# nghiahuynh-ai/Flamed-TTS

Hardware: AMD Instinct MI355X
Metric: latent frames/s (RTF at nsteps-denoiser=128) (higher is better)
Workload: dtype bf16; 1 GPU; BASELINE configs[1]: 1 utterance(s) x 400 frames (5.0 s audio) per GPU, nsteps-denoiser=128, bf16 (one persistent launch per solve); batch_per_gpu=1, frames=400, nfe=128, global_batch=1, parallelism=utterance-sharded x1 (no collectives)

## Files before the change

flamed-tts_amd/csrc/capi.cpp:

```cpp
#include <cstdarg>
#include <cstdio>
#include <cstring>
#include <mutex>

#include "common.hpp"
#include "flamed_hip.h"

namespace fl {
static thread_local char g_err[1024] = "";

void set_error(const char* fmt, ...) {
  va_list ap;
  va_start(ap, fmt);
  vsnprintf(g_err, sizeof(g_err), fmt, ap);
  va_end(ap);
}
const char* last_error() { return g_err; }

int device_of(const void* p, int* dev) {
  if (!p || !dev) return kBadArg;
  hipPointerAttribute_t a;
  if (hipPointerGetAttributes(&a, p) != hipSuccess) {
    (void)hipGetLastError();
    return kBadArg;
// ... 58 lines not shown
      {"dwgn_small", &Tune::dwgn_small, 0, 1, nullptr},
      {"fuse_euler", &Tune::fuse_euler, 0, 1, nullptr},
      {"pva_split", &Tune::pva_split, 0, 1, nullptr},
      {"persist", &Tune::persist, 0, 1, nullptr},
      {"split_batch", &Tune::split_batch, 1, 4, nullptr},
      {"split_graph", &Tune::split_graph, 0, 1, nullptr},
      {"split_prio", &Tune::split_prio, 0, 2, nullptr},
      {"prio_all", &Tune::prio_all, 0, 1, nullptr},
      {"split_min_rows", &Tune::split_min_rows, 1024, 1 << 30, nullptr},
      {"persist_opt", &Tune::persist_opt, 0, 1 << 20, nullptr},
      {"persist_seal_skip", &Tune::persist_seal_skip, -1, 1 << 20, nullptr},
      {"persist_inject", &Tune::persist_inject, -1, 1 << 20, nullptr},
      {"persist_multi", &Tune::persist_multi, 0, 1, nullptr},
      {"persist_pad", &Tune::persist_pad, 0, 1, nullptr},
      {"persist_pad_ntw", &Tune::persist_pad_ntw, 1, 8, nullptr},
      {"persist_multi_ntw", &Tune::persist_multi_ntw, 1, 8, nullptr},
      {"persist_ntw", &Tune::persist_ntw, 1, 8, nullptr},
      {"persist_capmode", &Tune::persist_capmode, 0, 1, nullptr},
      {"pva_persist", &Tune::pva_persist, 0, 1, nullptr},
      {"attn_mfma", &Tune::attn_mfma, 0, 1, nullptr},
      {"prior_split", &Tune::prior_split, 0, 1, nullptr},
      {"stop_after", &Tune::stop_after, -1, 1 << 20, nullptr},
      {"coop", &Tune::coop, 0, 1, nullptr},
      {"dwgn_var", &Tune::dwgn_var, 0, 2, nullptr},
      {"pva_stage", &Tune::pva_stage, 0, 3, nullptr},
      {"pva_inject", &Tune::pva_inject, -1, 1 << 20, nullptr},
  };
  for (const Knob& k : knobs) {
    if (std::strcmp(k.name, key) != 0) continue;
    int v = value;
// ... 30 lines not shown
```

flamed-tts_amd/csrc/common.hpp:

```cpp
#pragma once
#include <hip/hip_runtime.h>

#include <cstdint>
#include <cstdio>
#include <map>
#include <mutex>
#include <set>
#include <utility>
#include <vector>

namespace fl {

typedef __bf16 bf16;
typedef __bf16 bf16x8 __attribute__((ext_vector_type(8)));
typedef float f32x4 __attribute__((ext_vector_type(4)));
typedef unsigned int u32x4 __attribute__((ext_vector_type(4)));

void set_error(const char* fmt, ...);
const char* last_error();

enum Status : int {
  kOk = 0,
  kBadArg = 1001,
  kNoWorkspace = 1002,
// ... 126 lines not shown
  int x16 = 0;
  int g8p_rows = 12800;
  int dwgn = 1;
  int dwgn_small = 1;
  int fuse_euler = 1;
  int persist = 1;
  int split_batch = 2;
  int split_graph = 0;
  int prio_all = 0;
  int split_prio = 2;
  int split_min_rows = 6144;
  int persist_seal_skip = -1;
  int persist_inject = -1;
  int persist_pad = 1;
  int persist_pad_ntw = 4;
  int persist_multi = 1;
  int persist_ntw = 8;
  int persist_multi_ntw = 8;
  int persist_capmode = 0;
  int persist_opt = 885322;
  int pva_split = 0;
  int pva_persist = 1;
  int attn_mfma = 1;
  int prior_split = 1;
  int pva_stage = 1;
  int pva_inject = -1;
  int dwgn_var = 1;
  int coop = 1;
  int stop_after = -1;
};
// ... 165 lines not shown
```

flamed-tts_amd/csrc/denoiser.hip:

```cpp
#include <cstring>
#include "flamed_hip.h"
#include "flamed_diag.h"
#include "gemm.hpp"
#include "gemm_dma.hpp"
#include "gemm_8p.hpp"
#include "persist.hpp"

#include <mutex>
#include <string>
#include <vector>

namespace fl {

constexpr int kTinyRows = 320;

#ifdef FL_STAMPS
static unsigned long long* g_stamp_dev = nullptr;
static void stamp_select(int cls, hipStream_t st) {
  unsigned long long* p = (cls == tn().stamp_class) ? g_stamp_dev : nullptr;
  (void)hipMemcpyToSymbolAsync(HIP_SYMBOL(fl_stamp_buf), &p, sizeof(p), 0, hipMemcpyHostToDevice, st);
}
#else
static void stamp_select(int, hipStream_t) {}
#endif
// ... 1258 lines not shown
  if (idx >= R * dim) return;
  int r = idx / dim, j = idx - r * dim;
  int jj = j < half ? j : j - half;
  const float nl = -9.210340371976184f;
  float f = expf((nl * (float)jj) / (float)half);
  float a = t[r] * f;
  F[idx] = j < half ? cosf(a) : sinf(a);
}

__global__ void taps_t_kernel(const float* __restrict__ src, float* __restrict__ dst, int H, int KS) {
  const size_t i = (size_t)blockIdx.x * blockDim.x + threadIdx.x;
  if (i >= (size_t)H * KS) return;
  const int c = i / KS, j = i - (size_t)c * KS;
  dst[(size_t)j * H + c] = src[i];
}

__global__ void cast_kernel_bf16(const float* __restrict__ src, bf16* __restrict__ dst, size_t n) {
  size_t i = (size_t)blockIdx.x * blockDim.x + threadIdx.x;
  if (i < n) dst[i] = (bf16)src[i];
}
__global__ void copy_kernel_f32(const float* __restrict__ src, float* __restrict__ dst, size_t n) {
  size_t i = (size_t)blockIdx.x * blockDim.x + threadIdx.x;
  if (i < n) dst[i] = src[i];
}
template <typename DT>
__global__ void stack_taps_kernel(const float* __restrict__ src, DT* __restrict__ dst, int N, int Cin, int KT) {
  size_t i = (size_t)blockIdx.x * blockDim.x + threadIdx.x;
  size_t total = (size_t)N * Cin * KT;
  if (i >= total) return;
  int k = i % KT;
// ... 224 lines not shown
    return launch_gemm_cfg<32, 32, 3, DT>(al, W, ldw, ep, M, N, K, st);
  }
  if constexpr (std::is_same<DT, bf16>::value) {
    if (c == kCfgSmall && (tn().use_dma >= 2 || (tn().use_dma == 1 && AL::kSrcBytes == 2)))
      return launch_gemm_dma<32, 64>(al, W, ldw, ep, M, N, K, st);
  }
  return wide_a ? launch_gemm_auto<DT>(c, kWideA, al, W, ldw, ep, M, N, K, st) : launch_gemm_auto<DT>(c, al, W, ldw, ep, M, N, K, st);
}


struct DenBlockW {
  const void* w2; const void* w3; const void* m0; const void* m2;
  const unsigned char* q[4] = {nullptr, nullptr, nullptr, nullptr};
  const unsigned char* qs[4] = {nullptr, nullptr, nullptr, nullptr};
  const float *b2, *b3, *mb0, *mb2, *lnw, *lnb, *lnmw, *lnmb, *dww, *dwb, *gnw, *gnb;
};

struct Den {
  int C, H, NB, KS, S, dt;
  bool f8 = false;
  int MS;
  int MS0;
  int fold = 0;
  char* dev = nullptr;
  size_t dev_bytes = 0;
  float *t0w, *t0b, *t2w, *t2b, *cw, *cb, *adaw, *adab;
  void* win; const float* bin;
  std::vector<DenBlockW> blk;
  DenBlockW fin;
  void* wout; const float* bout;
// ... 278 lines not shown
  FL_ON_DEVICE(wdev);
  const int H = d->H, C = d->C, S = d->S, NB = d->NB, KS = d->KS;
  const size_t es = d->dt == FLAMED_BF16 ? 2 : 4;
  size_t off = 0;
  auto take = [&](size_t bytes) { size_t o = off; off = align256(off + bytes); return o; };
  size_t o_t0w = take(4ull * H * 256), o_t0b = take(4ull * H), o_t2w = take(4ull * H * H), o_t2b = take(4ull * H);
  size_t o_cw = take(4ull * H * S), o_cb = take(4ull * H);
  size_t o_adaw = take(4ull * d->MS0 * H), o_adab = take(4ull * d->MS0);
  size_t o_win = take(es * H * C);
  std::vector<size_t> o_blk(NB);
  for (int i = 0; i < NB; ++i) o_blk[i] = take(es * 4ull * H * H);
  size_t o_fin = take(es * 2ull * H * H);
  size_t o_out = take(es * (size_t)C * 3 * H);
  std::vector<size_t> o_dw(NB + 1);
  for (int i = 0; i <= NB; ++i) o_dw[i] = take(4ull * KS * H);
  const size_t n_vec = 1 + 11ull * NB + 5;
  const size_t o_vec = take(4ull * (n_vec * H + C));
  const size_t q_bytes = (size_t)H * H + mx_scale_bytes(H, H);
  const size_t o_q = d->f8 ? take(q_bytes * (4ull * NB + 2)) : 0;
  if (d->dev) { FL_HIP(hipFree(d->dev)); d->dev = nullptr; }
  FL_HIP(hipMalloc(&d->dev, off));
  d->dev_bytes = off;
  char* base = d->dev;
  auto cpy = [&](size_t o, const float* src, size_t n) -> int {
    hipLaunchKernelGGL(copy_kernel_f32, dim3((n + 255) / 256), dim3(256), 0, st, src, reinterpret_cast<float*>(base + o), n);
    FL_LAUNCH_CHECK();
    return kOk;
  };
  auto quant = [&](int slot, const float* src, const unsigned char** q, const unsigned char** qs) -> int {
    if (!d->f8) return kOk;
// ... 3 lines not shown
    FL_LAUNCH_CHECK();
    *q = p;
    *qs = p + (size_t)H * H;
    return kOk;
  };
  auto cast = [&](size_t o, const float* src, size_t n) -> int {
    if (d->dt == FLAMED_BF16) {
      hipLaunchKernelGGL(cast_kernel_bf16, dim3((n + 255) / 256), dim3(256), 0, st, src, reinterpret_cast<bf16*>(base + o), n);
      FL_LAUNCH_CHECK();
      return kOk;
    }
    return cpy(o, src, n);
  };
  int rc;
#define TRY(x) do { if ((rc = (x)) != kOk) return rc; } while (0)
  size_t vcur = o_vec;
  auto vec = [&](const float* src, size_t n, const float** dst) -> int {
    TRY(cpy(vcur, src, n));
    *dst = reinterpret_cast<const float*>(base + vcur);
    vcur += 4 * n;
    return kOk;
  };
  TRY(cpy(o_t0w, w[0], (size_t)H * 256)); TRY(cpy(o_t0b, w[1], H));
  TRY(cpy(o_t2w, w[2], (size_t)H * H)); TRY(cpy(o_t2b, w[3], H));
  TRY(cpy(o_cw, w[4], (size_t)H * S)); TRY(cpy(o_cb, w[5], H));
  TRY(cast(o_win, w[6], (size_t)H * C));
  d->t0w = (float*)(base + o_t0w); d->t0b = (float*)(base + o_t0b); d->t2w = (float*)(base + o_t2w); d->t2b = (float*)(base + o_t2b);
  d->cw = (float*)(base + o_cw); d->cb = (float*)(base + o_cb); d->adaw = (float*)(base + o_adaw); d->adab = (float*)(base + o_adab);
  d->win = base + o_win;
  TRY(vec(w[7], H, &d->bin));
// ... 2 lines not shown
    const float* const* bw = w + FLAMED_DEN_HEAD_W + FLAMED_DEN_BLOCK_W * i;
    TRY(cpy(o_adaw + 4ull * (size_t)i * 6 * H * H, bw[0], 6ull * H * H));
    TRY(cpy(o_adab + 4ull * (size_t)i * 6 * H, bw[1], 6ull * H));
    DenBlockW& B = d->blk[i];
    size_t ob = o_blk[i];
    TRY(cast(ob, bw[8], (size_t)H * H));
    TRY(cast(ob + es * H * H, bw[10], (size_t)H * H));
    TRY(cast(ob + 2 * es * H * H, bw[14], (size_t)H * H));
    TRY(cast(ob + 3 * es * H * H, bw[16], (size_t)H * H));
    B.w2 = base + ob; B.w3 = base + ob + es * H * H; B.m0 = base + ob + 2 * es * H * H; B.m2 = base + ob + 3 * es * H * H;
    TRY(quant(4 * i + 0, bw[8], &B.q[0], &B.qs[0])); TRY(quant(4 * i + 1, bw[10], &B.q[1], &B.qs[1]));
    TRY(quant(4 * i + 2, bw[14], &B.q[2], &B.qs[2])); TRY(quant(4 * i + 3, bw[16], &B.q[3], &B.qs[3]));
    hipLaunchKernelGGL(taps_t_kernel, dim3((H * KS + 255) / 256), dim3(256), 0, st, bw[4], reinterpret_cast<float*>(base + o_dw[i]), H, KS);
    FL_LAUNCH_CHECK();
    B.dww = reinterpret_cast<float*>(base + o_dw[i]);
    TRY(vec(bw[2], H, &B.lnw)); TRY(vec(bw[3], H, &B.lnb)); TRY(vec(bw[5], H, &B.dwb)); TRY(vec(bw[6], H, &B.gnw));
    TRY(vec(bw[7], H, &B.gnb)); TRY(vec(bw[9], H, &B.b2)); TRY(vec(bw[11], H, &B.b3)); TRY(vec(bw[12], H, &B.lnmw));
    TRY(vec(bw[13], H, &B.lnmb)); TRY(vec(bw[15], H, &B.mb0)); TRY(vec(bw[17], H, &B.mb2));
  }
  {
    const float* const* fw = w + FLAMED_DEN_HEAD_W + FLAMED_DEN_BLOCK_W * NB;
    TRY(cpy(o_adaw + 4ull * (size_t)NB * 6 * H * H, fw[0], 5ull * H * H));
    TRY(cpy(o_adab + 4ull * (size_t)NB * 6 * H, fw[1], 5ull * H));
    DenBlockW& F = d->fin;
    hipLaunchKernelGGL(taps_t_kernel, dim3((H * KS + 255) / 256), dim3(256), 0, st, fw[2], reinterpret_cast<float*>(base + o_dw[NB]), H, KS);
    FL_LAUNCH_CHECK();
    F.dww = reinterpret_cast<float*>(base + o_dw[NB]);
    TRY(vec(fw[3], H, &F.dwb)); TRY(vec(fw[4], H, &F.gnw)); TRY(vec(fw[5], H, &F.gnb));
    TRY(cast(o_fin, fw[6], (size_t)H * H)); TRY(vec(fw[7], H, &F.b2));
    TRY(cast(o_fin + es * H * H, fw[8], (size_t)H * H)); TRY(vec(fw[9], H, &F.b3));
    F.w2 = base + o_fin; F.w3 = base + o_fin + es * H * H;
    TRY(quant(4 * NB + 0, fw[6], &F.q[0], &F.qs[0])); TRY(quant(4 * NB + 1, fw[8], &F.q[1], &F.qs[1]));
    size_t n = (size_t)C * H * 3;
    if (d->dt == FLAMED_BF16)
      hipLaunchKernelGGL(stack_taps_kernel<bf16>, dim3((n + 255) / 256), dim3(256), 0, st, fw[10], reinterpret_cast<bf16*>(base + o_out), C, H, 3);
    else
      hipLaunchKernelGGL(stack_taps_kernel<float>, dim3((n + 255) / 256), dim3(256), 0, st, fw[10], reinterpret_cast<float*>(base + o_out), C, H, 3);
    FL_LAUNCH_CHECK();
    d->wout = base + o_out;
    TRY(vec(fw[11], C, &d->bout));
  }
#undef TRY
// ... 319 lines not shown
static size_t persist_layout(char* base, pk::Params* P) {
  size_t off = 0;
  auto take = [&](size_t bytes) { char* p = base ? base + off : nullptr; off = align256(off + bytes); return p; };
  const size_t T = pk::kMaxT, H = pk::kH, C = pk::kC;
  char* ctr = take(4 * (size_t)pk::kCtrInts);
  char* sticky = take(4 * (size_t)pk::kStickyInts);
  char* seal = take((size_t)pk::kWGs * 16);
  char* xp0 = take(T * pk::kSlots * 8);
  char* xp1 = take(T * pk::kSlots * 8);
  char* ximg = take(T * H * 4);
  char* a2 = take(T * H * 2);
  char* u = take(T * H * 2);
  char* xa = take(T * H * 2);
  char* xs = take(T * C * 2);
  char* gnp = take((size_t)pk::kGroups * H * 16);
  char* yb = take((size_t)pk::kWGs * 16 * 4);
  char* xbase = take(T * C * 4);
  if (P) {
    P->ctr = reinterpret_cast<int*>(ctr);
    P->sticky = reinterpret_cast<int*>(sticky);
    P->seal = reinterpret_cast<int*>(seal);
    P->xpart[0] = reinterpret_cast<float2*>(xp0);
    P->xpart[1] = reinterpret_cast<float2*>(xp1);
    P->ximg = reinterpret_cast<float*>(ximg);
    P->a2 = reinterpret_cast<bf16*>(a2);
    P->u = reinterpret_cast<bf16*>(u);
    P->xa = reinterpret_cast<bf16*>(xa);
    P->xs = reinterpret_cast<bf16*>(xs);
    P->gnp = reinterpret_cast<float4*>(gnp);
    P->yb = reinterpret_cast<float*>(yb);
    P->xbase = reinterpret_cast<float*>(xbase);
  }
  return off;
}

static int persist_alloc(Den* d, hipStream_t st) {
  if (d->pmem) return kOk;
  const size_t bytes = persist_layout(nullptr, nullptr);
  FL_HIP(hipMalloc(&d->pmem, bytes));
  FL_HIP(hipMemsetAsync(d->pmem, 0, bytes, st));
  FL_HIP(hipHostMalloc(reinterpret_cast<void**>(&d->pfail_host), 16, hipHostMallocDefault));
  *d->pfail_host = 0;
  FL_HIP(hipHostMalloc(reinterpret_cast<void**>(&d->perr_host), Den::kPRing * sizeof(int), hipHostMallocDefault));
  for (int i = 0; i < Den::kPRing; ++i) d->perr_host[i] = 0;
  d->pfails_seen = 0;
// ... 7 lines not shown

static void persist_poll_fails(Den* d) {
  if (!d->pfail_host) return;
  const int f = __atomic_load_n(d->pfail_host, __ATOMIC_RELAXED);
  if (f <= d->pfails_seen) return;
  d->pfails_seen = f;
  if (f >= Den::kPersistRetry && !d->pbroken) {
    d->pbroken = true;
    fprintf(stderr, "flamed: %d persistent solves failed (output NaN-poisoned); this handle uses the launch path from now on\n", f);
  } else {
    fprintf(stderr, "flamed: a persistent solve failed (%d of %d allowed); its output was NaN-poisoned\n", f, Den::kPersistRetry);
  }
}

static int persist_batch(int B) {
  if (B == 3) return 4;
  if (B >= 5 && B <= 7) return 8;
  return B;
}

static bool persist_eligible(Den* d, int B, int T) {
  const Tune& tu = tn();
  persist_poll_fails(d);
  if (!tu.persist || d->pbroken || d->dt != FLAMED_BF16 || d->f8 || !d->fold || !tu.lnfold) return false;
  if (d->H != pk::kH || d->C != pk::kC || d->NB > pk::kMaxNB || d->KS != pk::kTaps || T < 16) return false;
  const int B0 = B;
  if (B != 1 && tu.persist_multi && tu.persist_pad) B = persist_batch(B);
  if (B != 1 && (!tu.persist_multi || (B != 2 && B != 4 && B != 8))) return false;
  const int ntw = pk::persist_ntw(B, T, tu.persist_opt);
  if (B != B0 && 2 * B >= 3 * B0 && ntw > tu.persist_pad_ntw) return false;
  if (ntw > pk::kMaxNTW || ntw > tu.persist_ntw || ((tu.persist_opt & 1024) && ntw != 1)) return false;
  if (B > 1 && ntw > tu.persist_multi_ntw) return false;
  if (d->pdev_ok < 0) d->pdev_ok = pk::persist_device_ok(d->device) ? 1 : 0;
  return d->pdev_ok == 1;
}

struct Rk2 {
  double a;
  float dt, adt, c1, c2dt;
  Rk2(double a_, int nsteps) : a(a_) {
    const double h = 1.0 / (double)nsteps;
    dt = (float)h;
// ... 13 lines not shown
  const int Bp = tn().persist_pad ? persist_batch(B) : B;
  P.T = T; P.B = Bp; P.Bx = Bp != B ? B : 0; P.NB = d->NB; P.s0 = s0; P.s1 = s1;
  P.dt = (float)(1.0 / (double)nfe);
  if (rk) {
    P.rk2 = 1; P.dt = rk->dt; P.adt = rk->adt; P.c1 = rk->c1; P.c2dt = rk->c2dt;
  }
  P.mods = mods; P.MS = d->MS; P.MS0 = d->MS0;
  FL_REQUIRE(P.MS % 4 == 0 && P.MS0 % 4 == 0 && ((uintptr_t)mods & 15) == 0, "persistent solve: modulation rows not 16-B aligned");
  P.win = reinterpret_cast<const bf16*>(d->win); P.bin = d->bin;
  for (int i = 0; i <= d->NB; ++i) {
    const DenBlockW& b = i < d->NB ? d->blk[i] : d->fin;
    pk::BlockW& o = P.blk[i];
    o.w2 = reinterpret_cast<const bf16*>(b.w2); o.w3 = reinterpret_cast<const bf16*>(b.w3);
    o.m0 = i < d->NB ? reinterpret_cast<const bf16*>(b.m0) : nullptr;
    o.m2 = i < d->NB ? reinterpret_cast<const bf16*>(b.m2) : nullptr;
    o.b2 = b.b2; o.b3 = b.b3; o.dww = b.dww; o.dwb = b.dwb; o.gnw = b.gnw; o.gnb = b.gnb;
    if (i < d->NB) {
      o.mb0 = b.mb0; o.mb2 = b.mb2; o.lnw = b.lnw; o.lnb = b.lnb; o.lnmw = b.lnmw; o.lnmb = b.lnmb;
    }
  }
  P.wout = reinterpret_cast<const bf16*>(d->wout); P.bout = d->bout;
  P.xt = xt;
  P.tmo = 50000000;
  P.opt = tn().persist_opt;
  P.ntw = pk::persist_ntw(Bp, T, P.opt);
  P.inject_step = tn().persist_inject;
  P.seal_skip = tn().persist_seal_skip;
  hipEvent_t* ev = nullptr;
  const int slot = (int)(d->pring_n % Den::kPRing);
  if (!cap) {
// ... 531 lines not shown
```

flamed-tts_amd/csrc/persist.hip:

```cpp
#include <cstdio>
#include <cstdlib>

#include "flamed_hip.h"
#include "flamed_diag.h"
#include "persist.hpp"
#include "gemm_dma.hpp"

namespace fl {
namespace pk {

#ifdef FL_STAMPS
constexpr int kStampSlots = 160;
#define PST(step)                                                                                       \
  do {                                                                                                  \
    if ((step) == P.pst_step && P.pst && threadIdx.x == 0 && pst_k < kStampSlots)                       \
      P.pst[blockIdx.x * kStampSlots + pst_k] = __builtin_amdgcn_s_memrealtime();                      \
    ++pst_k;                                                                                            \
  } while (0)
#define PSTP(step) \
  (((step) == P.pst_step && P.pst && pst_k < kStampSlots) ? P.pst + blockIdx.x * kStampSlots + pst_k++ : (++pst_k, nullptr))
#define GND(k, v)                                                                                       \
  do {                                                                                                  \
    if (cur_step == P.gnd_step && P.gnd)                                                                \
      P.gnd[(((size_t)blk * kWGs + g * kSlots + s) * 32 + (tid & 31)) * 32 + (k)] = (v);                \
// ... 532 lines not shown

__device__ __forceinline__ void ld_cols(float (&v)[2][4], const float* p, int q) {
#pragma unroll
  for (int nt = 0; nt < 2; ++nt) {
    const float4 a = *reinterpret_cast<const float4*>(p + 16 * nt + 4 * q);
    v[nt][0] = a.x; v[nt][1] = a.y; v[nt][2] = a.z; v[nt][3] = a.w;
  }
}
__device__ __forceinline__ void fill_cols(float (&v)[2][4], float x) {
#pragma unroll
  for (int nt = 0; nt < 2; ++nt)
#pragma unroll
    for (int r = 0; r < 4; ++r) v[nt][r] = x;
}

__device__ __forceinline__ void row_stats(const float2* xpart, int T, int ra, int rb, int rbase, float* st) {
  const int n2 = 2 * (rb - ra);
  const __amdgpu_buffer_rsrc_t rs = rsrc(xpart, (unsigned)T * kSlots * 8);
  for (int idx = opq(threadIdx.x); idx < ((n2 + 63) & ~63); idx += kThreads) {
    const bool act = idx < n2;
    const int row = ra + (act ? idx >> 1 : 0), half = idx & 1;
    float mv[16], qv[16];
#pragma unroll
    for (int k = 0; k < 8; ++k) {
      const float4 v = as_f4(ld16(rs, (unsigned)((row * kSlots + half * 16 + 2 * k) * 8)));
      mv[2 * k] = v.x; qv[2 * k] = v.y; mv[2 * k + 1] = v.z; qv[2 * k + 1] = v.w;
    }
    float sm = 0.f;
#pragma unroll
    for (int k = 0; k < 16; ++k) sm += mv[k];
    sm = dpp_add<kDppXor1>(sm);
    const float mean = sm * (1.0f / kSlots);
    float m2 = 0.f;
#pragma unroll
    for (int k = 0; k < 16; ++k) {
      const float d = mv[k] - mean;
      m2 += qv[k] + (float)kCols * d * d;
    }
    m2 = dpp_add<kDppXor1>(m2);
    if (act && half == 0) {
      st[2 * (row - rbase)] = mean;
      st[2 * (row - rbase) + 1] = 1.0f / sqrtf(m2 * (1.0f / kH) + 1e-6f);
    }
  }
}

template <typename OT>
__device__ __forceinline__ void flush_tile(const char* stg, OT* dst, int ld, int r0, int ra, int rb, int col0, int T,
                                           bool local = false) {
  constexpr int CPR = kCols * (int)sizeof(OT) / 16;
  const __amdgpu_buffer_rsrc_t rs = rsrc(dst, (unsigned)T * ld * (unsigned)sizeof(OT));
  const int w16 = 16 * (threadIdx.x >> 6);
  for (int it = opq(threadIdx.x & 63); it < 16 * CPR; it += 64) {
    const int row = w16 + it / CPR, ch = it % CPR;
    if (row < ra || row >= rb) continue;
    const u32x4 v = *reinterpret_cast<const u32x4*>(stg + (row * kCols * sizeof(OT)) + ch * 16);
    const unsigned off = (unsigned)(((size_t)(r0 + row) * ld + col0) * sizeof(OT) + ch * 16);
    if (local) st16p(rs, off, v);
    else st16(rs, off, v);
// ... 35 lines not shown
__global__ __launch_bounds__(kThreads, 1) void den_persist_kernel(Params P) {
  extern __shared__ __attribute__((aligned(16))) char smem[];
  const int tid = threadIdx.x, lane = tid & 63;
  const int wave = __builtin_amdgcn_readfirstlane(tid >> 6);
  const int T = P.T;
  const int TT = P.B * P.T;
  const int H = kH;
  int g = blockIdx.x % kGroups, s = blockIdx.x / kGroups;
  if (P.opt & 8) {
    const int x = g, j = s;
    g = 4 * (x / 4) + (j % 4);
    s = 8 * (x % 4) + j / 4;
  }
  constexpr bool xloc = false;
  const bool frag = (P.opt & 64) != 0;
  const bool gran = (P.opt & 512) != 0;
  int r0, nr;
  group_rows(g, T, P.B, r0, nr, P.opt);
  const int gpu = kGroups / P.B, utt = g / gpu;
  const int ub = utt * T, ue = ub + T;
  const bool idle = P.Bx > 0 && utt >= P.Bx;
  const int MB = P.Bx > 0 ? P.Bx : P.B, mutt = idle ? P.Bx - 1 : utt;
  const int c = lane & 15, q = lane >> 4;
  const int col0 = kCols * s;
  char* stg = smem + L_HS;
  float* hs = reinterpret_cast<float*>(smem + L_HS);
  float* st = reinterpret_cast<float*>(smem + L_ST);
  float* red = reinterpret_cast<float*>(smem + L_RED);
  float4* gnv = reinterpret_cast<float4*>(smem + L_GNV);
  int* flag = reinterpret_cast<int*>(smem + L_FLAG);
// ... 150 lines not shown
    unsigned* const a1 = reinterpret_cast<unsigned*>(P.sticky + SY_ARRIVE1);
    unsigned* tk = reinterpret_cast<unsigned*>(smem + L_FLAG);
    if (tid == 0) tk[1] = __hip_atomic_fetch_add(a0, 1u, __ATOMIC_RELAXED, __HIP_MEMORY_SCOPE_AGENT);
    __syncthreads();
    const unsigned target = arrive_target(tk[1]);
    __syncthreads();
    const bool ok0 = arrive_wait(a0, target, tmo, flag);
    if (ok0) {
      if (tid < 4 && kCtrInts > 4 * (int)blockIdx.x + tid)
        __hip_atomic_store(P.ctr + 4 * blockIdx.x + tid, 0, __ATOMIC_RELAXED, __HIP_MEMORY_SCOPE_AGENT);
      if (tid < 4) __hip_atomic_store(P.seal + 4 * blockIdx.x + tid, 0, __ATOMIC_RELAXED, __HIP_MEMORY_SCOPE_AGENT);
      if (gran && tid < 32) {
        const __amdgpu_buffer_rsrc_t rq = rsrc(P.gnp, kGroups * kH * 16);
        st16(rq, (unsigned)((blockIdx.x * 32 + tid) * 16), u32x4{0u, 0u, 0u, 0u});
      }
      asm volatile("s_waitcnt vmcnt(0)" ::: "memory");
    }
    __syncthreads();
    if (tid == 0) __hip_atomic_fetch_add(a1, 1u, __ATOMIC_RELAXED, __HIP_MEMORY_SCOPE_AGENT);
    const bool ok1 = arrive_wait(a1, target, tmo, flag);
    if (!ok0 || !ok1) {
      if (tid == 0) {
        unsigned* pf = reinterpret_cast<unsigned*>(P.sticky + SY_PFAIL);
        if (__hip_atomic_exchange(pf, target, __ATOMIC_RELAXED, __HIP_MEMORY_SCOPE_AGENT) != target)
          __hip_atomic_fetch_add(fails, 1, __ATOMIC_RELAXED, __HIP_MEMORY_SCOPE_AGENT);
        __hip_atomic_store(errw, 5, __ATOMIC_RELAXED, __HIP_MEMORY_SCOPE_AGENT);
      }
      fail_exit();
      return;
    }
  }
  publish_xs();

  float X[NTW][2][4];

  for (int step = P.s0; step < P.s1; ++step) {
    const float* md = P.mods + (size_t)(step * MB + mutt) * P.MS;
    cur_step = step;
    if (step == P.inject_step) {
      if (tid == 0) raise_err(errw, fails, 3);
      fail_exit();
      return;
    }
#ifdef FL_STAMPS
    pst_k = 0;
#endif
    float binv[2][4];
// ... 26 lines not shown
      signal_dma<16>(mygrp);
    } else {
      signal(mygrp);
      next_w(P.blk[0].w2);
    }
    PST(step);
    ++L;

    for (int blk = 0; blk <= P.NB; ++blk) {
      const bool fin = blk == P.NB;
      const BlockW& bw = P.blk[blk];
      const float* mb = md + (size_t)blk * 6 * H;

      const int cc = tid & 31, rg = tid >> 5;
      float hsc[4], hsh[4], hlw[4], hlb[4], osc[2][4], osh[2][4], olw[2][4], olb[2][4];
#pragma unroll
      for (int e = 0; e < 4; ++e) {
        const int col = col0 + 4 * (tid & 7) + e;
        hsc[e] = mb[H + col];
        hsh[e] = mb[col];
        hlw[e] = fin ? 1.0f : bw.lnw[col];
        hlb[e] = fin ? 0.0f : bw.lnb[col];
      }
      ld_cols(osc, mb + H + col0, q);
      ld_cols(osh, mb + col0, q);
      if (fin) {
        fill_cols(olw, 1.0f);
        fill_cols(olb, 0.0f);
      } else {
        ld_cols(olw, bw.lnw + col0, q);
        ld_cols(olb, bw.lnb + col0, q);
      }
      float w[kTaps];
#pragma unroll
      for (int j = 0; j < kTaps; ++j) w[j] = bw.dww[(size_t)j * H + col0 + cc];
      const float dbias = bw.dwb[col0 + cc];
      float gwv = 0.f, gbv = 0.f;
      if (tid < kCols) {
        gwv = bw.gnw[col0 + tid];
        gbv = bw.gnb[col0 + tid];
      }
      PST(step);
      if (!wait_ge(errw, fails, tmo, grp, 16, kGroups, 32 * L, flag) || !seal_wait(0, kGroups)) { fail_exit(); return; }
      PST(step);
      float hva[4], hvb[4], ova[2][4], ovb[2][4];
#pragma unroll
      for (int e = 0; e < 4; ++e) {
        const float sc1 = 1.0f + hsc[e];
        hva[e] = fin ? sc1 : hlw[e] * sc1;
        hvb[e] = fin ? hsh[e] : hlb[e] * sc1 + hsh[e];
// ... 303 lines not shown
        signal(mygrp);
        if (fin) issue_out();
        else next_w(bw.m0);
      }
      PST(step);
      ++L;
      if (fin) break;

      const float* fo0 = md + P.MS0 + (size_t)blk * 2 * H;
      float fa0[2][4], fb0[2][4];
      ld_cols(fa0, fo0 + col0, q);
      ld_cols(fb0, fo0 + H + col0, q);
      PST(step);
      if (!wait_ge(errw, fails, tmo, mygrp, 0, 1, 32 * L, flag) || !seal_wait(g, 1)) { fail_exit(); return; }
      PST(step);
      row_stats(P.xpart[1], TT, r0, r0 + nr, r0 - kHalo, st);
      f32x4 accm_m0[NTW][2];
      if constexpr (KH) gemm_kh<kH>(P.xa, r0, nr, (smem + wb * kWPanel), accm_m0[0], wave, lane, PSTP(step), g, frag);
      else if constexpr (NTW == 1) gemm<kH>(P.xa, r0, nr, (smem + wb * kWPanel), accm_m0[0], wave, lane, PSTP(step), g, frag);
      else gemm_chunks<kH, NTW>(P.xa, r0, nr, (smem + wb * kWPanel), accm_m0, wave, lane, PSTP(step), g, frag, P.opt);
      PST(step);
#pragma unroll
      for (int ci = 0; ci < NTW; ++ci) {
        const int tl = wave + 4 * ci;
        const f32x4(&acc)[2] = accm_m0[ci];
        float v[2][4];
        const int p = 16 * tl + c + kHalo;
        const float mean = st[2 * p], rstd = st[2 * p + 1];
#pragma unroll
        for (int nt = 0; nt < 2; ++nt) {
#pragma unroll
          for (int i = 0; i < 4; ++i) v[nt][i] = silu(rstd * (acc[nt][i] - mean * fa0[nt][i]) + fb0[nt][i]);
        }
        if (16 * tl < nr) store_op_t(P.u, g, s, tl, v, r0, nr, col0, TT, lane, frag);
      }
      seal_put();
      if (dmafirst) {
        next_w(bw.m2);
        signal_dma<16>(mygrp);
      } else {
        signal(mygrp);
        next_w(bw.m2);
      }
// ... 40 lines not shown
    float fac[2][4], fbc[2][4];
    {
      const float* fo = md + P.MS0 + (size_t)P.NB * 2 * H;
#pragma unroll
      for (int nt = 0; nt < 2; ++nt) {
        const int n = 16 * nt + 4 * q, m = n < 24 ? n : n - 24;
        const int ns = (m >> 3) * kC + kCh * s + (m & 7);
        const float4 a = *reinterpret_cast<const float4*>(fo + ns), b = *reinterpret_cast<const float4*>(fo + 3 * kC + ns);
        fac[nt][0] = a.x; fac[nt][1] = a.y; fac[nt][2] = a.z; fac[nt][3] = a.w;
        fbc[nt][0] = b.x; fbc[nt][1] = b.y; fbc[nt][2] = b.z; fbc[nt][3] = b.w;
      }
    }
    PST(step);
    if (!wait_ge(errw, fails, tmo, mygrp, 0, 1, 32 * L, flag) || !seal_wait(g, 1)) { fail_exit(); return; }
    PST(step);
    row_stats(P.xpart[1], TT, r0, r0 + nr, r0 - kHalo, st);
    f32x4 acco[NTW][2];
    if constexpr (KH) gemm_kh<kH>(P.xa, r0, nr, (smem + wb * kWPanel), acco[0], wave, lane, PSTP(step), g, frag);
    else if constexpr (NTW == 1) gemm<kH>(P.xa, r0, nr, (smem + wb * kWPanel), acco[0], wave, lane, PSTP(step), g, frag);
    else gemm_chunks<kH, NTW>(P.xa, r0, nr, (smem + wb * kWPanel), acco, wave, lane, PSTP(step), g, frag, P.opt);
    PST(step);
    float* yl = reinterpret_cast<float*>(NTW == 1 ? stg : smem + wb * kWPanel);
    if (NTW > 1) __syncthreads();
#pragma unroll
    for (int ci = 0; ci < NTW; ++ci) {
      const int row = 16 * (wave + 4 * ci) + c, p = row + kHalo;
      if (NTW == 1 || row < nr) {
        const float mean = st[2 * p], rstd = st[2 * p + 1];
#pragma unroll
        for (int nt = 0; nt < 2; ++nt) {
          const int n0 = 16 * nt + 4 * q;
          if (n0 < 24) {
            float y[4];
#pragma unroll
            for (int i = 0; i < 4; ++i) y[i] = rstd * (acco[ci][nt][i] - mean * fac[nt][i]) + fbc[nt][i];
            *reinterpret_cast<float4*>(yl + row * 24 + n0) = make_float4(y[0], y[1], y[2], y[3]);
          }
        }
      }
    }
    __syncthreads();
    if (tid < 4 && nr > 0) {
      const __amdgpu_buffer_rsrc_t ry = rsrc(P.yb, kWGs * 16 * 4);
      const int half = tid >> 1, k = tid & 1;
      const float* src = half == 0 ? yl + (nr - 1) * 24 + 4 * k : yl + 16 + 4 * k;
      st16(ry, (unsigned)(((g + kGroups * s) * 16 + half * 8 + 4 * k) * 4), __builtin_bit_cast(u32x4, *reinterpret_cast<const float4*>(src)));
    }
    seal_put();
    if (dmafirst && step + 1 < P.s1) {
      next_win();
      signal_dma<4>(mygrp);
    } else {
      signal(mygrp);
      if (step + 1 < P.s1) next_win();
    }
    PST(step);
    ++L;

    PST(step);
    if (!wait_ge(errw, fails, tmo, grp, 16, kGroups, 32 * L, flag) || !seal_wait(0, kGroups)) { fail_exit(); return; }
    PST(step);
    int gp = 0, gn_ = 0;
    for (int k = 0; k < kGroups; ++k) {
      int a, b;
      group_rows(k, T, P.B, a, b, P.opt);
      if (b > 0 && a + b == r0) gp = k;
      if (b > 0 && a == r0 + nr) gn_ = k;
    }
#pragma unroll
    for (int ci = 0; ci < NTW; ++ci) {
      const int row = kChunk * ci + xr_row;
      if (row < nr) {
        const int t = r0 + row;
        const __amdgpu_buffer_rsrc_t ry = rsrc(P.yb, kWGs * 16 * 4);
        float vv[2];
#pragma unroll
        for (int e = 0; e < 2; ++e) {
          const int chl = 2 * (tid & 3) + e, ch = kCh * s + chl;
          float v = P.bout[ch] + yl[row * 24 + 8 + chl];
          if (t > ub) {
            const float y0 = row > 0 ? yl[(row - 1) * 24 + chl]
                                     : __builtin_bit_cast(float, __builtin_amdgcn_raw_buffer_load_b32(
                                           ry, (unsigned)(((gp + kGroups * s) * 16 + chl) * 4), 0, 16));
            v += y0;
          }
          if (t < ue - 1) {
            const float y2 = row < nr - 1 ? yl[(row + 1) * 24 + 16 + chl]
                                          : __builtin_bit_cast(float, __builtin_amdgcn_raw_buffer_load_b32(
                                                ry, (unsigned)(((gn_ + kGroups * s) * 16 + 8 + chl) * 4), 0, 16));
            v += y2;
          }
          vv[e] = v;
        }
        if constexpr (RK2) {
          float2* const stash = reinterpret_cast<float2*>(P.xbase + (size_t)t * kC + xch);
          if (!(step & 1)) {
            if constexpr (kStash) *stash = make_float2(xs0[ci], xs1[ci]);
            xs0[ci] = __fadd_rn(xs0[ci], __fmul_rn(P.adt, vv[0]));
            xs1[ci] = __fadd_rn(xs1[ci], __fmul_rn(P.adt, vv[1]));
          } else {
            float b0, b1;
            if constexpr (kStash) {
              const float2 b = *stash;
              b0 = b.x; b1 = b.y;
// ... 122 lines not shown
```

flamed-tts_amd/csrc/persist.hpp:

```cpp
#pragma once
#include "common.hpp"

namespace fl {
namespace pk {

constexpr int kGroups = 8, kSlots = 32, kWGs = kGroups * kSlots, kThreads = 256;
constexpr int kH = 1024, kC = 256, kCols = kH / kSlots, kCh = kC / kSlots;
constexpr int kChunk = 64, kMaxNTW = 8, kMaxRows = kChunk * kMaxNTW, kHalo = 15, kTaps = 31, kWin = kChunk + 2 * kHalo;
constexpr int kMaxNB = 8, kMaxT = kGroups * kMaxRows;
constexpr int kWPanel = kCols * kH * 2;
constexpr int kHsLd = kCols + 4;
constexpr int L_HS = 2 * kWPanel;
constexpr int L_ST = L_HS + kWin * kHsLd * 4;
constexpr int L_RED = L_ST + (kMaxRows + 2 * kHalo) * 8;
constexpr int L_GNV = L_RED + 8 * kCols * 4;
constexpr int L_FLAG = L_GNV + kCols * 16;
constexpr int kLds = (L_FLAG + 16 + 15) / 16 * 16;
static_assert(kLds <= 160 * 1024, "persistent solve LDS");
constexpr int CT_GRP = 0, CT_GN = 16 * kGroups, CT_ERR = CT_GN + 16 * kSlots, kCtrInts = CT_ERR + 16;
constexpr int SY_FAILS = 0, SY_ARRIVE0 = 32, SY_ARRIVE1 = 64, SY_PFAIL = 96, kStickyInts = 128;

__host__ __device__ inline unsigned arrive_target(unsigned ticket) {
  return ticket - ticket % (unsigned)kWGs + (unsigned)kWGs;
}
// ... 12 lines not shown
  const float* mods;
  int MS, MS0;
  const bf16* win;
  const float* bin;
  BlockW blk[kMaxNB + 1];
  const bf16* wout;
  const float* bout;
  float* xt;
  float2* xpart[2];
  float* ximg;
  bf16* a2;
  bf16* u;
  bf16* xa;
  bf16* xs;
  float4* gnp;
  float* yb;
  int* ctr;
  int* seal;
  int* sticky;
  int inject_step = -1;
  int seal_skip = -1;
  long long tmo;
  int ntw = 1;
  int opt = 0;
  unsigned long long* pst = nullptr;
  int pst_step = -1;
  float* gnd = nullptr;
  int gnd_step = -1;
  int rk2 = 0;
  float adt = 0.f, c1 = 0.f, c2dt = 0.f;
  float* xbase = nullptr;
};

bool persist_device_ok(int device);
inline int persist_ntw(int B, int T, int opt) {
  const int gpu = kGroups / B;
  int R = (T + gpu - 1) / gpu;
  if (opt & 2) R = ((T + 15) / 16 + gpu - 1) / gpu * 16;
  return (R + kChunk - 1) / kChunk;
}
int persist_launch(const Params& P, hipStream_t st, bool cooperative = true);

}
}
```

Measured before the change: 20400 latent frames/s.

## Replace group-wide barrier for output halo exchange with tagged per-neighbor atomics

The end-of-step output halo exchange no longer does a seal_put, a signal and a full wait across all groups. Each workgroup now publishes its boundary output rows as 64-bit tag+value atomics, and only the neighbor groups spin on those tags. The change also defers row-stat partial loads into registers for the NTW==1 path, so they overlap the GEMM instead of going through LDS. It adds a channel-major padded depthwise-tap copy for float4 loads, vectorises the modulation loads for NTW<=4, and adds an optional batch-padding knob. The spin-wait removes the global barrier but relies on tag ordering being correct, so a wrong tag could cause stale reads or hangs.

Result: faster. 21210 latent frames/s (median of 6 runs) (+4.0%).

```diff
diff --git a/flamed-tts_amd/csrc/capi.cpp b/flamed-tts_amd/csrc/capi.cpp
--- a/flamed-tts_amd/csrc/capi.cpp
+++ b/flamed-tts_amd/csrc/capi.cpp
@@ -96,6 +96,7 @@
       {"persist_multi", &Tune::persist_multi, 0, 1, nullptr},
       {"persist_pad", &Tune::persist_pad, 0, 1, nullptr},
       {"persist_pad_ntw", &Tune::persist_pad_ntw, 1, 8, nullptr},
+      {"persist_as", &Tune::persist_as, 0, 8, nullptr},
       {"persist_multi_ntw", &Tune::persist_multi_ntw, 1, 8, nullptr},
       {"persist_ntw", &Tune::persist_ntw, 1, 8, nullptr},
       {"persist_capmode", &Tune::persist_capmode, 0, 1, nullptr},
diff --git a/flamed-tts_amd/csrc/common.hpp b/flamed-tts_amd/csrc/common.hpp
--- a/flamed-tts_amd/csrc/common.hpp
+++ b/flamed-tts_amd/csrc/common.hpp
@@ -164,6 +164,7 @@
   int persist_inject = -1;
   int persist_pad = 1;
   int persist_pad_ntw = 4;
+  int persist_as = 0;
   int persist_multi = 1;
   int persist_ntw = 8;
   int persist_multi_ntw = 8;
diff --git a/flamed-tts_amd/csrc/denoiser.hip b/flamed-tts_amd/csrc/denoiser.hip
--- a/flamed-tts_amd/csrc/denoiser.hip
+++ b/flamed-tts_amd/csrc/denoiser.hip
@@ -1296,6 +1296,12 @@
   const int c = i / KS, j = i - (size_t)c * KS;
   dst[(size_t)j * H + c] = src[i];
 }
+__global__ void taps_cm_kernel(const float* __restrict__ src, float* __restrict__ dst, int H, int KS) {
+  const size_t i = (size_t)blockIdx.x * blockDim.x + threadIdx.x;
+  if (i >= (size_t)H * 32) return;
+  const int c = i / 32, j = i % 32;
+  dst[i] = j < KS ? src[(size_t)c * KS + j] : 0.f;
+}
 
 __global__ void cast_kernel_bf16(const float* __restrict__ src, bf16* __restrict__ dst, size_t n) {
   size_t i = (size_t)blockIdx.x * blockDim.x + threadIdx.x;
@@ -1550,6 +1556,7 @@
   const unsigned char* q[4] = {nullptr, nullptr, nullptr, nullptr};
   const unsigned char* qs[4] = {nullptr, nullptr, nullptr, nullptr};
   const float *b2, *b3, *mb0, *mb2, *lnw, *lnb, *lnmw, *lnmb, *dww, *dwb, *gnw, *gnb;
+  const float* dwc = nullptr;
 };
 
 struct Den {
@@ -1858,6 +1865,8 @@
   size_t o_out = take(es * (size_t)C * 3 * H);
   std::vector<size_t> o_dw(NB + 1);
   for (int i = 0; i <= NB; ++i) o_dw[i] = take(4ull * KS * H);
+  std::vector<size_t> o_dwc(NB + 1);
+  for (int i = 0; i <= NB; ++i) o_dwc[i] = take(4ull * 32 * H);
   const size_t n_vec = 1 + 11ull * NB + 5;
   const size_t o_vec = take(4ull * (n_vec * H + C));
   const size_t q_bytes = (size_t)H * H + mx_scale_bytes(H, H);
@@ -1891,6 +1900,14 @@
   };
   int rc;
 #define TRY(x) do { if ((rc = (x)) != kOk) return rc; } while (0)
+  auto taps_cm = [&](size_t o, const float* src, const float** dst) -> int {
+    *dst = nullptr;
+    if (KS > 32) return kOk;
+    hipLaunchKernelGGL(taps_cm_kernel, dim3((H * 32 + 255) / 256), dim3(256), 0, st, src, reinterpret_cast<float*>(base + o), H, KS);
+    FL_LAUNCH_CHECK();
+    *dst = reinterpret_cast<const float*>(base + o);
+    return kOk;
+  };
   size_t vcur = o_vec;
   auto vec = [&](const float* src, size_t n, const float** dst) -> int {
     TRY(cpy(vcur, src, n));
@@ -1923,6 +1940,7 @@
     hipLaunchKernelGGL(taps_t_kernel, dim3((H * KS + 255) / 256), dim3(256), 0, st, bw[4], reinterpret_cast<float*>(base + o_dw[i]), H, KS);
     FL_LAUNCH_CHECK();
     B.dww = reinterpret_cast<float*>(base + o_dw[i]);
+    TRY(taps_cm(o_dwc[i], bw[4], &B.dwc));
     TRY(vec(bw[2], H, &B.lnw)); TRY(vec(bw[3], H, &B.lnb)); TRY(vec(bw[5], H, &B.dwb)); TRY(vec(bw[6], H, &B.gnw));
     TRY(vec(bw[7], H, &B.gnb)); TRY(vec(bw[9], H, &B.b2)); TRY(vec(bw[11], H, &B.b3)); TRY(vec(bw[12], H, &B.lnmw));
     TRY(vec(bw[13], H, &B.lnmb)); TRY(vec(bw[15], H, &B.mb0)); TRY(vec(bw[17], H, &B.mb2));
@@ -1935,6 +1953,7 @@
     hipLaunchKernelGGL(taps_t_kernel, dim3((H * KS + 255) / 256), dim3(256), 0, st, fw[2], reinterpret_cast<float*>(base + o_dw[NB]), H, KS);
     FL_LAUNCH_CHECK();
     F.dww = reinterpret_cast<float*>(base + o_dw[NB]);
+    TRY(taps_cm(o_dwc[NB], fw[2], &F.dwc));
     TRY(vec(fw[3], H, &F.dwb)); TRY(vec(fw[4], H, &F.gnw)); TRY(vec(fw[5], H, &F.gnb));
     TRY(cast(o_fin, fw[6], (size_t)H * H)); TRY(vec(fw[7], H, &F.b2));
     TRY(cast(o_fin + es * H * H, fw[8], (size_t)H * H)); TRY(vec(fw[9], H, &F.b3));
@@ -2284,7 +2303,7 @@
   char* xa = take(T * H * 2);
   char* xs = take(T * C * 2);
   char* gnp = take((size_t)pk::kGroups * H * 16);
-  char* yb = take((size_t)pk::kWGs * 16 * 4);
+  char* yb = take((size_t)pk::kWGs * 2 * pk::kCh * 8);
   char* xbase = take(T * C * 4);
   if (P) {
     P->ctr = reinterpret_cast<int*>(ctr);
@@ -2298,7 +2317,7 @@
     P->xa = reinterpret_cast<bf16*>(xa);
     P->xs = reinterpret_cast<bf16*>(xs);
     P->gnp = reinterpret_cast<float4*>(gnp);
-    P->yb = reinterpret_cast<float*>(yb);
+    P->yb = reinterpret_cast<unsigned long long*>(yb);
     P->xbase = reinterpret_cast<float*>(xbase);
   }
   return off;
@@ -2336,6 +2355,8 @@
 }
 
 static int persist_batch(int B) {
+  const int as = tn().persist_as;
+  if ((as == 2 || as == 4 || as == 8) && B < as) return as;
   if (B == 3) return 4;
   if (B >= 5 && B <= 7) return 8;
   return B;
@@ -2347,7 +2368,7 @@
   if (!tu.persist || d->pbroken || d->dt != FLAMED_BF16 || d->f8 || !d->fold || !tu.lnfold) return false;
   if (d->H != pk::kH || d->C != pk::kC || d->NB > pk::kMaxNB || d->KS != pk::kTaps || T < 16) return false;
   const int B0 = B;
-  if (B != 1 && tu.persist_multi && tu.persist_pad) B = persist_batch(B);
+  if (tu.persist_multi && tu.persist_pad) B = persist_batch(B);
   if (B != 1 && (!tu.persist_multi || (B != 2 && B != 4 && B != 8))) return false;
   const int ntw = pk::persist_ntw(B, T, tu.persist_opt);
   if (B != B0 && 2 * B >= 3 * B0 && ntw > tu.persist_pad_ntw) return false;
@@ -2391,6 +2412,7 @@
     o.w2 = reinterpret_cast<const bf16*>(b.w2); o.w3 = reinterpret_cast<const bf16*>(b.w3);
     o.m0 = i < d->NB ? reinterpret_cast<const bf16*>(b.m0) : nullptr;
     o.m2 = i < d->NB ? reinterpret_cast<const bf16*>(b.m2) : nullptr;
+    P.dwc[i] = b.dwc;
     o.b2 = b.b2; o.b3 = b.b3; o.dww = b.dww; o.dwb = b.dwb; o.gnw = b.gnw; o.gnb = b.gnb;
     if (i < d->NB) {
       o.mb0 = b.mb0; o.mb2 = b.mb2; o.lnw = b.lnw; o.lnb = b.lnb; o.lnmw = b.lnmw; o.lnmb = b.lnmb;
diff --git a/flamed-tts_amd/csrc/persist.hip b/flamed-tts_amd/csrc/persist.hip
--- a/flamed-tts_amd/csrc/persist.hip
+++ b/flamed-tts_amd/csrc/persist.hip
@@ -570,35 +570,64 @@
     for (int r = 0; r < 4; ++r) v[nt][r] = x;
 }
 
+template <class PairAdd>
+__device__ __forceinline__ float2 combine_row_partials(const float (&mv)[16], const float (&qv)[16], PairAdd pair) {
+  float sm = 0.f;
+#pragma unroll
+  for (int k = 0; k < 16; ++k) sm += mv[k];
+  sm = pair(sm);
+  const float mean = sm * (1.0f / kSlots);
+  float m2 = 0.f;
+#pragma unroll
+  for (int k = 0; k < 16; ++k) {
+    const float d = mv[k] - mean;
+    m2 += qv[k] + (float)kCols * d * d;
+  }
+  m2 = pair(m2);
+  return make_float2(mean, 1.0f / sqrtf(m2 * (1.0f / kH) + 1e-6f));
+}
+__device__ __forceinline__ void unpack_row_partials(const u32x4 (&v)[8], float (&mv)[16], float (&qv)[16]) {
+#pragma unroll
+  for (int k = 0; k < 8; ++k) {
+    const float4 f = as_f4(v[k]);
+    mv[2 * k] = f.x; qv[2 * k] = f.y; mv[2 * k + 1] = f.z; qv[2 * k + 1] = f.w;
+  }
+}
+
 __device__ __forceinline__ void row_stats(const float2* xpart, int T, int ra, int rb, int rbase, float* st) {
   const int n2 = 2 * (rb - ra);
   const __amdgpu_buffer_rsrc_t rs = rsrc(xpart, (unsigned)T * kSlots * 8);
   for (int idx = opq(threadIdx.x); idx < ((n2 + 63) & ~63); idx += kThreads) {
     const bool act = idx < n2;
     const int row = ra + (act ? idx >> 1 : 0), half = idx & 1;
+    u32x4 v[8];
+#pragma unroll
+    for (int k = 0; k < 8; ++k) v[k] = ld16(rs, (unsigned)((row * kSlots + half * 16 + 2 * k) * 8));
     float mv[16], qv[16];
-#pragma unroll
-    for (int k = 0; k < 8; ++k) {
-      const float4 v = as_f4(ld16(rs, (unsigned)((row * kSlots + half * 16 + 2 * k) * 8)));
-      mv[2 * k] = v.x; qv[2 * k] = v.y; mv[2 * k + 1] = v.z; qv[2 * k + 1] = v.w;
-    }
-    float sm = 0.f;
-#pragma unroll
-    for (int k = 0; k < 16; ++k) sm += mv[k];
-    sm = dpp_add<kDppXor1>(sm);
-    const float mean = sm * (1.0f / kSlots);
-    float m2 = 0.f;
-#pragma unroll
-    for (int k = 0; k < 16; ++k) {
-      const float d = mv[k] - mean;
-      m2 += qv[k] + (float)kCols * d * d;
-    }
-    m2 = dpp_add<kDppXor1>(m2);
+    unpack_row_partials(v, mv, qv);
+    const float2 ms = combine_row_partials(mv, qv, [](float x) { return dpp_add<kDppXor1>(x); });
     if (act && half == 0) {
-      st[2 * (row - rbase)] = mean;
-      st[2 * (row - rbase) + 1] = 1.0f / sqrtf(m2 * (1.0f / kH) + 1e-6f);
-    }
-  }
+      st[2 * (row - rbase)] = ms.x;
+      st[2 * (row - rbase) + 1] = ms.y;
+    }
+  }
+}
+
+__device__ __forceinline__ void load_row_partials(u32x4 (&v)[8], const float2* xpart, int T, int r0, int nr, int tile,
+                                                  int lane_in) {
+  const int lane = opq(lane_in);
+  const int c = lane & 15, q = lane >> 4, row = 16 * tile + c;
+  const __amdgpu_buffer_rsrc_t rs = rsrc(xpart, (unsigned)T * kSlots * 8);
+  const unsigned base = q < 2 && row < nr ? (unsigned)(((r0 + row) * kSlots + q * 16) * 8) : 0x7ff00000u;
+#pragma unroll
+  for (int k = 0; k < 8; ++k) v[k] = ld16(rs, base + 16 * k);
+}
+__device__ __forceinline__ float2 finish_row_partials(const u32x4 (&v)[8], int lane_in) {
+  float mv[16], qv[16];
+  unpack_row_partials(v, mv, qv);
+  const float2 ms = combine_row_partials(mv, qv, [](float x) { return x + __shfl_xor(x, 16); });
+  const int c = lane_in & 15;
+  return make_float2(__shfl(ms.x, c), __shfl(ms.y, c));
 }
 
 template <typename OT>
@@ -664,6 +693,7 @@
   }
   constexpr bool xloc = false;
   const bool frag = (P.opt & 64) != 0;
+  constexpr bool kDefer = NTW == 1 && !KH;
   const bool gran = (P.opt & 512) != 0;
   int r0, nr;
   group_rows(g, T, P.B, r0, nr, P.opt);
@@ -844,6 +874,10 @@
         const __amdgpu_buffer_rsrc_t rq = rsrc(P.gnp, kGroups * kH * 16);
         st16(rq, (unsigned)((blockIdx.x * 32 + tid) * 16), u32x4{0u, 0u, 0u, 0u});
       }
+      if (tid < 8) {
+        const __amdgpu_buffer_rsrc_t ry = rsrc(P.yb, kWGs * 2 * kCh * 8);
+        st16(ry, (unsigned)((blockIdx.x * 8 + tid) * 16), u32x4{0u, 0u, 0u, 0u});
+      }
       asm volatile("s_waitcnt vmcnt(0)" ::: "memory");
     }
     __syncthreads();
@@ -861,6 +895,16 @@
     }
   }
   publish_xs();
+
+  unsigned long long* const ybq = P.yb;
+  int gp = 0, gn_ = 0;
+  for (int k = 0; k < kGroups; ++k) {
+    int a, b;
+    group_rows(k, T, P.B, a, b, P.opt);
+    if (b > 0 && a + b == r0) gp = k;
+    if (b > 0 && a == r0 + nr) gn_ = k;
+  }
+  const bool ynb_p = !idle && nr > 0 && r0 > ub, ynb_n = !idle && nr > 0 && r0 + nr < ue;
 
   float X[NTW][2][4];
 
@@ -917,13 +961,28 @@
 
       const int cc = tid & 31, rg = tid >> 5;
       float hsc[4], hsh[4], hlw[4], hlb[4], osc[2][4], osh[2][4], olw[2][4], olb[2][4];
-#pragma unroll
-      for (int e = 0; e < 4; ++e) {
-        const int col = col0 + 4 * (tid & 7) + e;
-        hsc[e] = mb[H + col];
-        hsh[e] = mb[col];
-        hlw[e] = fin ? 1.0f : bw.lnw[col];
-        hlb[e] = fin ? 0.0f : bw.lnb[col];
+      constexpr bool kWide = NTW <= 4;
+      if constexpr (!kWide) {
+#pragma unroll
+        for (int e = 0; e < 4; ++e) {
+          const int col = col0 + 4 * (tid & 7) + e;
+          hsc[e] = mb[H + col];
+          hsh[e] = mb[col];
+          hlw[e] = fin ? 1.0f : bw.lnw[col];
+          hlb[e] = fin ? 0.0f : bw.lnb[col];
+        }
+      } else {
+        const int col = col0 + 4 * (tid & 7);
+        const float4 a = *reinterpret_cast<const float4*>(mb + H + col), b = *reinterpret_cast<const float4*>(mb + col);
+        hsc[0] = a.x; hsc[1] = a.y; hsc[2] = a.z; hsc[3] = a.w;
+        hsh[0] = b.x; hsh[1] = b.y; hsh[2] = b.z; hsh[3] = b.w;
+        float4 lw = make_float4(1.0f, 1.0f, 1.0f, 1.0f), lb = make_float4(0.0f, 0.0f, 0.0f, 0.0f);
+        if (!fin) {
+          lw = *reinterpret_cast<const float4*>(bw.lnw + col);
+          lb = *reinterpret_cast<const float4*>(bw.lnb + col);
+        }
+        hlw[0] = lw.x; hlw[1] = lw.y; hlw[2] = lw.z; hlw[3] = lw.w;
+        hlb[0] = lb.x; hlb[1] = lb.y; hlb[2] = lb.z; hlb[3] = lb.w;
       }
       ld_cols(osc, mb + H + col0, q);
       ld_cols(osh, mb + col0, q);
@@ -935,8 +994,18 @@
         ld_cols(olb, bw.lnb + col0, q);
       }
       float w[kTaps];
-#pragma unroll
-      for (int j = 0; j < kTaps; ++j) w[j] = bw.dww[(size_t)j * H + col0 + cc];
+      if constexpr (kWide) {
+        const float4* wp = reinterpret_cast<const float4*>(P.dwc[blk] + (size_t)(col0 + cc) * 32);
+#pragma unroll
+        for (int j = 0; j < 8; ++j) {
+          const float4 t = wp[j];
+          w[4 * j] = t.x; w[4 * j + 1] = t.y; w[4 * j + 2] = t.z;
+          if (4 * j + 3 < kTaps) w[4 * j + 3] = t.w;
+        }
+      } else {
+#pragma unroll
+        for (int j = 0; j < kTaps; ++j) w[j] = bw.dww[(size_t)j * H + col0 + cc];
+      }
       const float dbias = bw.dwb[col0 + cc];
       float gwv = 0.f, gbv = 0.f;
       if (tid < kCols) {
@@ -1270,7 +1339,9 @@
       PST(step);
       if (!wait_ge(errw, fails, tmo, mygrp, 0, 1, 32 * L, flag) || !seal_wait(g, 1)) { fail_exit(); return; }
       PST(step);
-      row_stats(P.xpart[1], TT, r0, r0 + nr, r0 - kHalo, st);
+      [[maybe_unused]] u32x4 rp_m0[8];
+      if constexpr (kDefer) load_row_partials(rp_m0, P.xpart[1], TT, r0, nr, wave, lane);
+      else row_stats(P.xpart[1], TT, r0, r0 + nr, r0 - kHalo, st);
       f32x4 accm_m0[NTW][2];
       if constexpr (KH) gemm_kh<kH>(P.xa, r0, nr, (smem + wb * kWPanel), accm_m0[0], wave, lane, PSTP(step), g, frag);
       else if constexpr (NTW == 1) gemm<kH>(P.xa, r0, nr, (smem + wb * kWPanel), accm_m0[0], wave, lane, PSTP(step), g, frag);
@@ -1281,8 +1352,16 @@
         const int tl = wave + 4 * ci;
         const f32x4(&acc)[2] = accm_m0[ci];
         float v[2][4];
-        const int p = 16 * tl + c + kHalo;
-        const float mean = st[2 * p], rstd = st[2 * p + 1];
+        float mean, rstd;
+        if constexpr (kDefer) {
+          const float2 ms = finish_row_partials(rp_m0, lane);
+          mean = ms.x;
+          rstd = ms.y;
+        } else {
+          const int p = 16 * tl + c + kHalo;
+          mean = st[2 * p];
+          rstd = st[2 * p + 1];
+        }
 #pragma unroll
         for (int nt = 0; nt < 2; ++nt) {
 #pragma unroll
@@ -1353,7 +1432,9 @@
     PST(step);
     if (!wait_ge(errw, fails, tmo, mygrp, 0, 1, 32 * L, flag) || !seal_wait(g, 1)) { fail_exit(); return; }
     PST(step);
-    row_stats(P.xpart[1], TT, r0, r0 + nr, r0 - kHalo, st);
+    [[maybe_unused]] u32x4 rp_out[8];
+    if constexpr (kDefer) load_row_partials(rp_out, P.xpart[1], TT, r0, nr, wave, lane);
+    else row_stats(P.xpart[1], TT, r0, r0 + nr, r0 - kHalo, st);
     f32x4 acco[NTW][2];
     if constexpr (KH) gemm_kh<kH>(P.xa, r0, nr, (smem + wb * kWPanel), acco[0], wave, lane, PSTP(step), g, frag);
     else if constexpr (NTW == 1) gemm<kH>(P.xa, r0, nr, (smem + wb * kWPanel), acco[0], wave, lane, PSTP(step), g, frag);
@@ -1365,7 +1446,15 @@
     for (int ci = 0; ci < NTW; ++ci) {
       const int row = 16 * (wave + 4 * ci) + c, p = row + kHalo;
       if (NTW == 1 || row < nr) {
-        const float mean = st[2 * p], rstd = st[2 * p + 1];
+        float mean, rstd;
+        if constexpr (kDefer) {
+          const float2 ms = finish_row_partials(rp_out, lane);
+          mean = ms.x;
+          rstd = ms.y;
+        } else {
+          mean = st[2 * p];
+          rstd = st[2 * p + 1];
+        }
 #pragma unroll
         for (int nt = 0; nt < 2; ++nt) {
           const int n0 = 16 * nt + 4 * q;
@@ -1379,54 +1468,64 @@
       }
     }
     __syncthreads();
-    if (tid < 4 && nr > 0) {
-      const __amdgpu_buffer_rsrc_t ry = rsrc(P.yb, kWGs * 16 * 4);
-      const int half = tid >> 1, k = tid & 1;
-      const float* src = half == 0 ? yl + (nr - 1) * 24 + 4 * k : yl + 16 + 4 * k;
-      st16(ry, (unsigned)(((g + kGroups * s) * 16 + half * 8 + 4 * k) * 4), __builtin_bit_cast(u32x4, *reinterpret_cast<const float4*>(src)));
-    }
-    seal_put();
-    if (dmafirst && step + 1 < P.s1) {
-      next_win();
-      signal_dma<4>(mygrp);
-    } else {
-      signal(mygrp);
-      if (step + 1 < P.s1) next_win();
-    }
+    const unsigned ytag = (unsigned)(step - P.s0 + 1);
+    if (tid < 2 * kCh && nr > 0 && !idle) {
+      const float y = tid < kCh ? yl[(nr - 1) * 24 + tid] : yl[16 + tid - kCh];
+      __hip_atomic_store(ybq + (size_t)(g + kGroups * s) * (2 * kCh) + tid, ((unsigned long long)ytag << 32) | __float_as_uint(y),
+                         __ATOMIC_RELAXED, __HIP_MEMORY_SCOPE_AGENT);
+    }
+    if (step + 1 < P.s1) next_win();
     PST(step);
-    ++L;
 
     PST(step);
-    if (!wait_ge(errw, fails, tmo, grp, 16, kGroups, 32 * L, flag) || !seal_wait(0, kGroups)) { fail_exit(); return; }
+    if (ynb_p || ynb_n) {
+      if (tid < 64) {
+        const bool need = tid < kCh ? ynb_p : tid < 2 * kCh && ynb_n;
+        const unsigned long long* yq = ybq + (size_t)((tid < kCh ? gp : gn_) + kGroups * s) * (2 * kCh) + (tid & (2 * kCh - 1));
+        float y = 0.f;
+        bool ok = true;
+        const unsigned long long t0 = __builtin_amdgcn_s_memrealtime();
+        for (unsigned it = 0;; ++it) {
+          bool mine = true;
+          if (need) {
+            const unsigned long long a = __hip_atomic_load(yq, __ATOMIC_RELAXED, __HIP_MEMORY_SCOPE_AGENT);
+            mine = (unsigned)(a >> 32) == ytag;
+            y = __uint_as_float((unsigned)a);
+          }
+          if (__all(mine)) break;
+          if ((it & 31) == 31) {
+            if (__hip_atomic_load(errw, __ATOMIC_RELAXED, __HIP_MEMORY_SCOPE_AGENT) != 0) { ok = false; break; }
+            if ((long long)(__builtin_amdgcn_s_memrealtime() - t0) > tmo) {
+              if (tid == 0) raise_err(errw, fails, 1);
+              ok = false;
+              break;
+            }
+          }
+          __builtin_amdgcn_s_sleep(1);
+        }
+        if (tid == 0) *flag = ok ? 1 : 0;
+        if (tid < 2 * kCh) red[tid] = y;
+      }
+      __syncthreads();
+      if (*flag == 0) { fail_exit(); return; }
+    }
     PST(step);
-    int gp = 0, gn_ = 0;
-    for (int k = 0; k < kGroups; ++k) {
-      int a, b;
-      group_rows(k, T, P.B, a, b, P.opt);
-      if (b > 0 && a + b == r0) gp = k;
-      if (b > 0 && a == r0 + nr) gn_ = k;
-    }
 #pragma unroll
     for (int ci = 0; ci < NTW; ++ci) {
       const int row = kChunk * ci + xr_row;
       if (row < nr) {
         const int t = r0 + row;
-        const __amdgpu_buffer_rsrc_t ry = rsrc(P.yb, kWGs * 16 * 4);
         float vv[2];
 #pragma unroll
         for (int e = 0; e < 2; ++e) {
           const int chl = 2 * (tid & 3) + e, ch = kCh * s + chl;
           float v = P.bout[ch] + yl[row * 24 + 8 + chl];
           if (t > ub) {
-            const float y0 = row > 0 ? yl[(row - 1) * 24 + chl]
-                                     : __builtin_bit_cast(float, __builtin_amdgcn_raw_buffer_load_b32(
-                                           ry, (unsigned)(((gp + kGroups * s) * 16 + chl) * 4), 0, 16));
+            const float y0 = row > 0 ? yl[(row - 1) * 24 + chl] : ynb_p ? red[chl] : 0.f;
             v += y0;
           }
           if (t < ue - 1) {
-            const float y2 = row < nr - 1 ? yl[(row + 1) * 24 + 16 + chl]
-                                          : __builtin_bit_cast(float, __builtin_amdgcn_raw_buffer_load_b32(
-                                                ry, (unsigned)(((gn_ + kGroups * s) * 16 + 8 + chl) * 4), 0, 16));
+            const float y2 = row < nr - 1 ? yl[(row + 1) * 24 + 16 + chl] : ynb_n ? red[kCh + chl] : 0.f;
             v += y2;
           }
           vv[e] = v;
diff --git a/flamed-tts_amd/csrc/persist.hpp b/flamed-tts_amd/csrc/persist.hpp
--- a/flamed-tts_amd/csrc/persist.hpp
+++ b/flamed-tts_amd/csrc/persist.hpp
@@ -50,7 +50,7 @@
   bf16* xa;
   bf16* xs;
   float4* gnp;
-  float* yb;
+  unsigned long long* yb;
   int* ctr;
   int* seal;
   int* sticky;
@@ -66,6 +66,7 @@
   int rk2 = 0;
   float adt = 0.f, c1 = 0.f, c2dt = 0.f;
   float* xbase = nullptr;
+  const float* dwc[kMaxNB + 1] = {};
 };
 
 bool persist_device_ok(int device);
```
